# ZijiaLewisLu/CVPR2025-DeCafNet

Hardware: AMD Instinct MI355X
Metric: clips/sec (grounding fwd, T=16384 D=1024) (higher is better)
Workload: dtype f32; 1 GPU; BASELINE configs[2]: T=16384 D=1024 full multi-scale pyramid + sidekick top-k 30% + expert path, NQ=1 queries/video, 24 independent videos per step: 3 forwards in flight on 3 HIP streams x 8 videos per forward, one replica of this per GPU; T=16384, vid_len=16384, D=1024, E=256, TE=256, levels=8, win=9, heads=4, fusion_layers=2, sn=60, msf=True, norm=True, Lq=32, nq=1, max_batch=8, forwards_in_flight=3

## Files before the change

cvpr2025-decafnet_amd/_lib.py:

```python
import ctypes
import os

_HERE = os.path.dirname(os.path.abspath(__file__))
SO_PATH = os.environ.get('DCF_LIB_PATH') or os.path.join(_HERE, 'libdecafnet_hip.so')
_LIB = None

c_f32p = ctypes.c_void_p
c_u8p = ctypes.c_void_p
c_i32p = ctypes.c_void_p
c_i64p = ctypes.c_void_p
i32, i64, f32, f64 = ctypes.c_int32, ctypes.c_int64, ctypes.c_float, ctypes.c_double
vp = ctypes.c_void_p


class DcfConfig(ctypes.Structure):
    _fields_ = [(n, i32) for n in ('D', 'E', 'TE', 'vid_heads', 'fusion_heads', 'fusion_layers', 'n_embd_convs',
                                   'n_stem', 'n_levels', 'win', 'head_layers', 'sn')] + \
               [('sratio', f32)] + [(n, i32) for n in ('msf', 'norm', 'use_abs_pe', 'max_batch', 'gemm_mode', 'model_kind', 'second_fusion',
                                                      'text_in', 'text_layers', 'text_heads', 'text_abs_pe', 'text_bkgd',
                                                      'scat', 'sfonly', 'text_kind', 'xattn_affine', 'vid_stride', 'pool_only', 'attn_mode')]


SIGNATURES = {
    'dcf_last_error': (ctypes.c_char_p, []),
# ... 34 lines not shown
    'dcf_hybrid_phase2': (i32, [vp, c_f32p, c_u8p, i64, c_f32p, vp]),
    'dcf_hybrid_phase3': (i32, [vp, c_f32p, c_f32p, c_f32p, c_u8p, c_f32p, c_f32p, c_u8p, vp]),
    'dcf_debug_copy': (i32, [vp, i32, c_f32p, i64, vp]),
    'dcf_graph_active': (i32, [vp]),
    'dcf_debug_set_option': (i32, [ctypes.c_char_p, i32]),
    'dcf_calib_mfma_rate': (i32, [i32, i32, ctypes.POINTER(i32), ctypes.POINTER(f32)]),
    'dcf_model_set_graph_mode': (i32, [vp, i32]),
    'dcf_model_set_ln_carry': (i32, [vp, i32]),
    'dcf_profile_enable': (i32, [i32]),
    'dcf_profile_report': (i64, [ctypes.c_char_p, i64]),
    'dcf_collect_segments': (i32, [c_f32p, c_f32p, c_u8p, i32, i64, i32, f32, i32, f32, c_f32p, c_f32p, c_i32p, vp]),
    'dcf_collect_segments_ext': (i32, [c_f32p, c_f32p, c_u8p, c_f32p, i32, i64, i32, f32, i32, f32, c_f32p, c_f32p, c_i32p, vp]),
    'dcf_nms_1d': (i32, [c_f32p, c_f32p, c_i32p, i32, i32, i32, f32, c_i64p, c_i32p, vp]),
    'dcf_softnms_1d': (i32, [c_f32p, c_f32p, c_i32p, i32, i32, i32, f32, f32, f32, i32, i32, c_f32p, c_i64p, c_i32p, vp]),
    'dcf_segment_voting': (i32, [c_f32p, i32, c_i32p, i32, i32, c_f32p, c_f32p, c_i32p, i32, i32, f32, i32, c_f32p, vp]),
    'dcf_op_linear': (i32, [c_f32p, c_f32p, c_f32p, c_f32p, i32, i32, i32, i32, vp]),
    'dcf_op_linear_split': (i32, [c_f32p, c_f32p, c_f32p, c_f32p, i32, i32, i32, i32, i32, vp]),
    'dcf_op_linear_cm': (i32, [c_f32p, c_f32p, c_f32p, c_f32p, i32, i32, i32, vp]),
    'dcf_op_linear_ln': (i32, [c_f32p, c_f32p, c_f32p, c_f32p, c_f32p, c_f32p, c_f32p, i32, i32, i32, i32, i32, vp]),
    'dcf_op_linear_ln_carry': (i32, [c_f32p, c_f32p, c_f32p, c_f32p, c_f32p, c_f32p, c_f32p, c_f32p, c_f32p, c_f32p, i32, i32, i32, i32, i32, i32, vp]),
    'dcf_op_ffn': (i32, [c_f32p, c_f32p, c_f32p, c_f32p, c_f32p, c_f32p, c_f32p, c_f32p, c_u8p, c_f32p, c_f32p, i32, i32, i32, vp]),
    'dcf_op_linear_cm_split': (i32, [c_f32p, c_f32p, c_f32p, c_f32p, i32, i32, i32, i32, vp]),
    'dcf_op_head': (i32, [c_f32p, c_u8p, c_f32p, c_f32p, c_f32p, c_f32p, c_f32p, c_f32p, c_f32p, c_f32p, c_f32p, i32, i32, i32, i32, f32, i32, vp]),
    'dcf_op_conv3': (i32, [c_f32p, c_u8p, c_f32p, c_f32p, i32, i32, i32, i32, vp]),
    'dcf_op_conv3_split': (i32, [c_f32p, c_u8p, c_f32p, c_f32p, i32, i32, i32, i32, i32, vp]),
    'dcf_op_layernorm': (i32, [c_f32p, c_f32p, c_f32p, c_f32p, i32, i32, i32, vp]),
    'dcf_op_xattn': (i32, [c_f32p, c_f32p, c_f32p, c_u8p, c_f32p, i32, i32, i32, i32, i32, vp]),
    'dcf_op_local_attn': (i32, [c_f32p, c_f32p, c_f32p, c_u8p, c_f32p, i32, i32, i32, i32, i32, vp]),
    'dcf_op_sidekick': (i32, [c_f32p, c_f32p, c_f32p, i32, i32, i32, i32, vp]),
    'dcf_op_gate': (i32, [c_f32p, c_u8p, c_f32p, c_u8p, i32, i32, i32, f64, i32, vp]),
    'dcf_op_encoder': (i32, [vp, ctypes.c_char_p, c_f32p, c_u8p, i32, i32, i32, c_f32p, c_u8p, vp]),
    'dcf_op_enc_pre': (i32, [vp, ctypes.c_char_p, c_f32p, c_u8p, i32, i32, i32, c_f32p, c_f32p, c_f32p, c_f32p, vp]),
    'dcf_op_decoder': (i32, [vp, ctypes.c_char_p, c_f32p, c_u8p, i32, i32, ctypes.POINTER(vp), ctypes.POINTER(vp), ctypes.POINTER(i32), vp]),
    'dcf_op_tcn': (i32, [vp, ctypes.c_char_p, c_f32p, c_u8p, i32, i32, i32, i32, c_f32p, vp]),
}


def lib():
    global _LIB
    if _LIB is None:
        import torch
        if not os.path.exists(SO_PATH):
            raise RuntimeError(f'{SO_PATH} is missing: build it with __graft_entry__.build() '
                               f'(there is no CPU fallback for the grounding path)')
        h = ctypes.CDLL(SO_PATH, mode=ctypes.RTLD_GLOBAL)
        for name, (res, args) in SIGNATURES.items():
# ... 21 lines not shown
```

cvpr2025-decafnet_amd/csrc/engine.hip:

```cpp
#include <cstdarg>
#include <cstdio>
#include <cstdlib>
#include <algorithm>
#include <cstring>
#include <string>
#include <atomic>
#include <mutex>
#include <unordered_map>
#include <vector>

#include "../../include/decafnet_hip.h"
#include "attn.h"
#include "common.h"
#include "dec_chain.h"
#include "dropout.h"
#include "enc_chain.h"
#include "ffn_chain.h"
#include "gemm.h"
#include "head_chain.h"
#include "heads.h"
#include "postproc.h"
#include "rowops.h"
#include "score.h"

// ... 126 lines not shown
  const float *fc_wf, *fc_s, *fc_c;
  const unsigned short* qkv_chain[3];
  const float *qkv_s[3], *qkv_c[3];
  const unsigned short* wp_chain;
};
struct DecW {
  const float *ln_q_w, *ln_q_b, *ln_kv_w, *ln_kv_b, *dw, *qn_w, *qn_b;
  const float *wq, *bq, *wk, *bk, *wv, *bv, *wp, *bp;
  const float *wp_il, *bp_il;
  const float *ln_ffn_w, *ln_ffn_b, *fc_w, *fc_b, *pj_w, *pj_b, *ls_ffn;
  const float *fc_wf, *fc_s, *fc_c;
  const unsigned short *wq_chain, *wp_chain;
};
struct TextEncW {
  const float *ln_attn_w, *ln_attn_b, *wq, *bq, *wk, *bk, *wv, *bv, *wp, *bp, *ls_attn;
  const float *ln_ffn_w, *ln_ffn_b, *fc_w, *fc_b, *pj_w, *pj_b, *ls_ffn;
};
struct HeadW {
  std::vector<const float*> conv;
  std::vector<const float*> ln_w, ln_b;
  const float* out_w;
  const float* out_b;
  const unsigned short* chain[2] = {nullptr, nullptr};
};

static inline int vid_stride_of(const dcf_config& c) { return c.vid_stride > 1 ? c.vid_stride : 1; }

struct Plan {
  int T0 = 0, B = 0, L = 0;
  LevelTable lt{};
  LevelTable* d_lt = nullptr;
};

}

using namespace dcf;

namespace dcf { struct HybridState; }
using dcf::HybridState;

struct dcf_model {
  dcf_config cfg{};
  std::unordered_map<std::string, Bound> bound;
  std::vector<float*> owned;
  std::unordered_map<const float*, const unsigned short*> wsplit;
  std::unordered_map<const float*, int64_t> wsplit_ldw;
// ... 294 lines not shown
  for (int i = 0; i < layers; ++i) {
    const std::string s = std::to_string(i);
    GET(p + ".convs." + s + ".conv.weight", SH(C, C, 3), t);
    const float* pk;
    if (pack3(m, t, C, C, 3, 0, 2, 1, st, &pk)) return -1;
    SPLIT(pk, C, 3 * C);
    h.conv.push_back(pk);
    const float *lw, *lb;
    GET(p + ".norms." + s + ".weight", SH(C), lw); GET(p + ".norms." + s + ".bias", SH(C), lb);
    h.ln_w.push_back(lw); h.ln_b.push_back(lb);
  }
  GET(p + "." + out_name + ".conv.weight", SH(NO, C, 3), t);
  if (pack3(m, t, NO, C, 3, 0, 2, 1, st, &h.out_w)) return -1;
  GET(p + "." + out_name + ".conv.bias", SH(NO), h.out_b);
  h.chain[0] = h.chain[1] = nullptr;
  if (m->gemm_terms == GEMM_F16X3 && layers == 2 && head_chain_supports(C, NO)) {
    for (int i = 0; i < 2; ++i) {
      unsigned short* img = nullptr;
      DCF_HIP(hipMalloc(&img, head_chain_image_halfs(C) * sizeof(unsigned short)));
      m->owned.push_back(reinterpret_cast<float*>(img));
      if (launch_split_chain3(h.conv[i], img, C, st, nullptr)) return -1;
      h.chain[i] = img;
    }
  }
  return 0;
}

static inline bool vidmap_sfonly(const dcf_config& c) { return c.model_kind == 0 && c.msf && c.sfonly; }
static inline int vidmap_in_dim(const dcf_config& c) {
  return ((c.msf && !vidmap_sfonly(c)) ? 2 * c.D : c.D) + (c.scat ? 1 : 0);
}

static int finalize(dcf_model* m, hipStream_t st) {
  const dcf_config& c = m->cfg;
  const int E = c.E, D = c.D, TE = c.TE, L = c.n_levels;
  const bool sfonly = vidmap_sfonly(c);
  const int Din = vidmap_in_dim(c);
  for (float* p : m->owned) (void)hipFree(p);
  m->owned.clear();
  m->wsplit.clear();
  m->wsplit_ldw.clear();
  m->wsplit_terms.clear();
  if (init_gemm_mode(m, st)) return -1;
  m->dec.clear(); m->stem.clear(); m->branch.clear();
  m->embd_conv.clear(); m->embd_ln_w.clear(); m->embd_ln_b.clear();
  m->cls1 = HeadW(); m->cls2 = HeadW(); m->reg = HeadW();
// ... 403 lines not shown
  }
  GemmArgs gp = gemm(b.R[0], E, w.wp, w.bp, b.R[1], E, rows, E, E);
  gp.flags = G_RES | G_RES_MASK; gp.rowmask = mask_out; gp.ls = w.ls_attn;
  if (stride == 2) { gp.R = b.R[3]; gp.ldr = E; } else { gp.R = Xin; gp.ldr = ldx; }
  GemmArgs go = gemm(b.HID, 4 * E, w.pj_w, w.pj_b, Xout, ldo, rows, E, 4 * E);
  go.flags = G_RES | G_OUT_MASK; go.rowmask = mask_out; go.ls = w.ls_ffn; go.R = b.R[1]; go.ldr = E;
  if (can_fuse_ln(m, w.wp, rows, E, E, A_ROWS)) {
    gp.ln_w = w.ln_ffn_w; gp.ln_b = w.ln_ffn_b; gp.Y = b.R[2]; gp.ldy = E;
    TRY(run_gemm(m, &gp, 1, A_ROWS, st));
  } else if (can_carry_ln(m, w.wp, w.fc_wf, rows, E, E, E)) {
    gp.stats_out = b.stats; gp.stats_w = STATS_W;
    TRY(run_gemm(m, &gp, 1, A_ROWS, st));
    return run_ffn(m, b.R[1], w.fc_wf, w.fc_c, go, b.HID, rows, E, st, b.stats, w.fc_s);
  } else {
    TRY(run_gemm(m, &gp, 1, A_ROWS, st));
    LnArgs ln{}; ln.X = b.R[1]; ln.ldx = E; ln.Y = b.R[2]; ln.ldy = E; ln.w = w.ln_ffn_w; ln.b = w.ln_ffn_b; ln.rows = rows; ln.C = E;
    TRY(launch_ln(ln, st));
  }
  TRY(run_ffn(m, b.R[2], w.fc_w, w.fc_b, go, b.HID, rows, E, st));
  return 0;
}

static int head_chain_min_rows() {
  static const int v = getenv("DCF_HEAD_CHAIN_MIN_ROWS") ? atoi(getenv("DCF_HEAD_CHAIN_MIN_ROWS")) : 30000;
  return v;
}
static bool g_no_head_chain() {
  static const bool off = getenv("DCF_NO_HEAD_CHAIN") != nullptr;
  return off;
}
static bool can_chain_head(dcf_model* m, const HeadW& h, int rows, int Cin, int NO) {
  if (g_no_head_chain() || rows < head_chain_min_rows() || m->gemm_terms != GEMM_F16X3 || !h.chain[0] || !h.chain[1]) return false;
  if (h.conv.size() != 2 || !head_chain_supports(Cin, NO)) return false;
  for (int i = 0; i < 2; ++i)
    if (!m->wsplit.count(h.conv[i]) || m->wsplit_terms[h.conv[i]] != GEMM_F16X3) return false;
  return true;
}
static HeadChainArgs head_chain_args(dcf_model* m, const HeadW& h, Buffers& b, const Plan& pl, int NO, int mode, int query_major, float* out) {
  HeadChainArgs a{};
  a.X = b.F; a.ldx = m->cfg.E + TCN_HID; a.nbr = b.nbr_all; a.W1c = h.chain[0]; a.W2c = h.chain[1];
  a.ln1_w = h.ln_w[0]; a.ln1_b = h.ln_b[0]; a.ln2_w = h.ln_w[1]; a.ln2_b = h.ln_b[1];
  a.Wout = h.out_w; a.bout = h.out_b; a.lt = pl.d_lt; a.out = out; a.rows = pl.B * pl.lt.S; a.NO = NO; a.mode = mode;
  a.query_major = query_major; a.status = m->status;
  return a;
}
static int run_head_chain(dcf_model* m, const HeadChainArgs* a, int count, int Cin, hipStream_t st) {
  double flops = 0., bytes = 0.;
  for (int i = 0; i < count; ++i) {
    flops += 2.0 * a[i].rows * Cin * 3.0 * Cin * 2.0 + 2.0 * a[i].rows * 3.0 * Cin * a[i].NO;
    bytes += (double)a[i].rows * (Cin + a[i].NO) * 4.0;
  }
  ProfScope prof("gemm_f16x3<head_chain>", st, flops, bytes);
  return launch_head_chain(a, count, Cin, st);
}

static int run_head(dcf_model* m, const HeadW& h, Buffers& b, const Plan& pl, int Cin, int NO, int mode, int query_major,
                    float* out, hipStream_t st, int row0 = 0, int rows = -1) {
  if (row0 == 0 && rows < 0 && can_chain_head(m, h, pl.B * pl.lt.S, Cin, NO)) {
    const HeadChainArgs a = head_chain_args(m, h, b, pl, NO, mode, query_major, out);
    return run_head_chain(m, &a, 1, Cin, st);
  }
  const int rowsAll = rows >= 0 ? rows : pl.B * pl.lt.S;
  const int ldf = m->cfg.E + TCN_HID;
  const float* in = b.F + (int64_t)row0 * ldf;
  int64_t ldin = ldf;
// ... 1217 lines not shown
}

int dcf_hybrid_phase2(dcf_model* m, const float* featk_c, const uint8_t* maskk_c, int64_t off_k, float* refk_out, void* stream) {
  DCF_CHECK(m && featk_c && maskk_c && refk_out, "dcf_hybrid_phase2: null argument");
  DCF_CHECK(m->hyb && m->hyb->valid, "dcf_hybrid_phase2: no phase 1 on this model (or another forward ran since)");
  DCF_CHECK(off_k >= 0 && off_k + (m->hyb->Tn >> m->hyb->k) <= m->hyb->Tc, "dcf_hybrid_phase2: the narrow window must lie inside the coarse one");
  return dcf::hybrid_phase2(m, featk_c, maskk_c, (int)off_k, refk_out, (hipStream_t)stream);
}

int dcf_hybrid_phase3(dcf_model* m, const float* refk_c, float* logits_n, float* offsets_n, uint8_t* masks_n, float* logits_c,
                      float* offsets_c, uint8_t* masks_c, void* stream) {
  DCF_CHECK(m && refk_c && logits_n && offsets_n && masks_n, "dcf_hybrid_phase3: null argument");
  DCF_CHECK(m->hyb && m->hyb->valid, "dcf_hybrid_phase3: no phase 1 / 2 on this model (or another forward ran since)");
  DCF_CHECK(m->cfg.n_levels - m->hyb->k <= 1 || (logits_c && offsets_c && masks_c), "dcf_hybrid_phase3: null coarse outputs");
  const int rc = dcf::hybrid_phase3(m, refk_c, logits_n, offsets_n, masks_n, logits_c, offsets_c, masks_c, (hipStream_t)stream);
  m->hyb->valid = false;
  return rc;
}

int dcf_graph_active(const dcf_model* m) { return m ? m->last_launch : 0; }

int dcf_debug_set_option(const char* name, int32_t value) {
  DCF_CHECK(name && *name, "dcf_debug_set_option: empty name");
  static const char* known[] = {"dec_chain_min_rows", "enc_chain_min_rows", "enc_attn_min_rows", "fuse_scores", "tcn_frag", "gate_skip", "tcn_stack"};
  bool ok = false;
  for (const char* k : known) ok = ok || strcmp(k, name) == 0;
  DCF_CHECK(ok, "dcf_debug_set_option: unknown option '%s'", name);
  {
    std::lock_guard<std::mutex> lock(dcf::debug_options_mutex());
    if (value < 0) dcf::debug_options().erase(name);
    else dcf::debug_options()[name] = value;
  }
  dcf::g_option_epoch.fetch_add(1);
  return 0;
}

int dcf_model_set_graph_mode(dcf_model* m, int32_t mode) {
  DCF_CHECK(m && mode >= 0 && mode <= 2, "dcf_model_set_graph_mode: mode must be 0 (auto), 1 (always) or 2 (never)");
  if (mode != m->graph_mode) dcf::drop_graph(m);
  m->graph_mode = mode;
  return 0;
}

int dcf_debug_copy(dcf_model* m, int32_t what, float* dst, int64_t max_floats, void* stream) {
  DCF_CHECK(m && dst, "dcf_debug_copy: null argument");
  hipStream_t st = (hipStream_t)stream;
  const float* src = nullptr;
// ... 372 lines not shown
      dcf::GemmArgs g = dcf::gemm(in, C, wp[i], nullptr, bufs[i], C, rows, C, 3 * C);
      g.cin = C; g.nbr = nbr; g.Ws = img[i];
      rc = dcf::launch_gemm_split(&g, 1, dcf::A_ROWS_TAP3, nterms, st);
      if (rc == 0) {
        dcf::LnArgs ln{}; ln.X = bufs[i]; ln.ldx = C; ln.Y = bufs[i]; ln.ldy = C; ln.w = lw[i]; ln.b = lb[i]; ln.rows = rows; ln.C = C; ln.relu = 1;
        rc = dcf::launch_ln(ln, st);
      }
      in = bufs[i];
    }
    if (rc == 0) {
      dcf::ConvOutArgs co{};
      co.X = in; co.ldx = C; co.nbr = nbr; co.W = wo; co.bias = bout; co.lt = d_lt; co.out = out; co.rows = rows; co.C = C; co.NO = NO;
      co.row0 = 0; co.mode = mode; co.query_major = 0;
      rc = dcf::launch_conv_out(co, st);
    }
  }
  for (int i = 0; i < 2; ++i) { if (wp[i]) DCF_HIP(hipFreeAsync(wp[i], st)); if (img[i]) DCF_HIP(hipFreeAsync(img[i], st)); }
  if (ha) DCF_HIP(hipFreeAsync(ha, st));
  if (hb) DCF_HIP(hipFreeAsync(hb, st));
  DCF_HIP(hipFreeAsync(wo, st)); DCF_HIP(hipFreeAsync(nbr, st)); DCF_HIP(hipFreeAsync(d_lt, st));
  return rc;
}

int dcf_op_layernorm(const float* X, const float* w, const float* b, float* Y, int32_t rows, int32_t C, int32_t relu,
                     void* stream) {
  dcf::LnArgs a{};
  a.X = X; a.ldx = C; a.Y = Y; a.ldy = C; a.w = w; a.b = b; a.rows = rows; a.C = C; a.relu = relu;
  return dcf::launch_ln(a, (hipStream_t)stream);
}

int dcf_op_xattn(const float* Q, const float* K, const float* V, const uint8_t* kvmask, float* O, int32_t B, int32_t T,
                 int32_t Lk, int32_t C, int32_t heads, void* stream) {
  dcf::XAttnArgs a{Q, K, V, kvmask, O, B, T, Lk, C, heads};
  return dcf::launch_xattn(a, (hipStream_t)stream);
}

int dcf_op_local_attn(const float* Q, const float* K, const float* V, const uint8_t* mask, float* O, int32_t B, int32_t T,
                      int32_t C, int32_t heads, int32_t window, void* stream) {
  if (window == 0) {
    dcf::GlobalAttnArgs g{Q, K, V, mask, O, B, T, C, heads};
    return dcf::launch_global_attn(g, (hipStream_t)stream);
  }
  dcf::LocalAttnArgs a{Q, K, V, mask, O, B, T, C, heads, window};
  return dcf::launch_local_attn(a, (hipStream_t)stream);
}

// ... 150 lines not shown
```

cvpr2025-decafnet_amd/csrc/head_chain.h:

```cpp
#pragma once
#include <hip/hip_runtime.h>
#include <stdint.h>

#include "heads.h"

namespace dcf {

struct HeadChainArgs {
  const float* X;
  int64_t ldx;
  const uint8_t* nbr;
  const unsigned short* W1c;
  const unsigned short* W2c;
  const float* ln1_w; const float* ln1_b; const float* ln2_w; const float* ln2_b;
  const float* Wout;
  const float* bout;
  const LevelTable* lt;
  float* out;
  int rows, NO;
  int mode;
  int query_major;
  unsigned* status;
};

bool head_chain_supports(int C, int NO);
int launch_head_chain(const HeadChainArgs* a, int count, int C, hipStream_t stream);
size_t head_chain_image_halfs(int C);
int launch_split_chain3(const float* Wp, unsigned short* img, int C, hipStream_t stream, unsigned* overflow = nullptr);

}
```

cvpr2025-decafnet_amd/csrc/head_chain.hip:

```cpp
#include "head_chain.h"

#include <type_traits>

#include "common.h"

namespace dcf {

namespace {

typedef _Float16 f16x8 __attribute__((ext_vector_type(8)));
typedef _Float16 f16x2 __attribute__((ext_vector_type(2)));
typedef float f32x2 __attribute__((ext_vector_type(2)));
typedef unsigned u32x4 __attribute__((ext_vector_type(4)));

constexpr float SA = 16.f, SW = 256.f, UNSCALE = 1.f / 4096.f;
constexpr int HALO = 3, WGROWS = 128, VALID = WGROWS - 2 * HALO;

template <int C>
struct Geo {
  static constexpr int KS = C / 16;
  static constexpr int KH = KS / 2;
  static constexpr int NT = C / 32;
  static constexpr int PIECES = 3 * KH * 2;
  static constexpr int STAGE = PIECES * 1024;
  static constexpr int SPL = 2 * NT;
  static constexpr int NPW = (PIECES + 3) / 4;
  static_assert(C % 32 == 0 && KS % 2 == 0, "C must be a multiple of 32");
};

__device__ __forceinline__ void split2_f16(float x0, float x1, float s, unsigned& hi, unsigned& lo) {
  const f16x2 h = __builtin_convertvector(f32x2{x0 * s, x1 * s}, f16x2);
  hi = __builtin_bit_cast(unsigned, h);
  const float r0 = __builtin_fmaf(x0, s, -(float)h[0]), r1 = __builtin_fmaf(x1, s, -(float)h[1]);
  lo = __builtin_bit_cast(unsigned, __builtin_convertvector(f32x2{r0, r1}, f16x2));
}

__device__ __forceinline__ void glds16(const void* sbase, unsigned voff, unsigned lds_dst) {
#ifdef DCF_GLDS_KEEP_M0
  unsigned keep;
// ... 33 lines not shown

}

template <int C>
__global__ void k_split_chain3(const float* __restrict__ Wp, unsigned short* __restrict__ img, unsigned* __restrict__ overflow) {
  using G = Geo<C>;
  const int i = blockIdx.x * blockDim.x + threadIdx.x;
  if (i >= C * 3 * (C / 2)) return;
  const int n = i / (3 * (C / 2)), rem = i - n * (3 * (C / 2)), tap = rem / (C / 2), k = (rem - tap * (C / 2)) * 2;
  const float w0 = Wp[((size_t)n * 3 + tap) * C + k], w1 = Wp[((size_t)n * 3 + tap) * C + k + 1];
  unsigned hi, lo;
  split2_f16(w0, w1, SW, hi, lo);
  if (!(__builtin_fabsf(w0) * SW <= 65504.f) || !(__builtin_fabsf(w1) * SW <= 65504.f)) {
    if (overflow) atomicOr(overflow, 1u);
  }
  const int ot = n >> 5, rr = n & 31, kk = k >> 4, hf = kk / G::KH, kq = kk - hf * G::KH, kr = k & 15;
  const int a = kr >> 3, h = (kr >> 2) & 1, ii = kr & 3, j = 4 * a + ii;
  const size_t piece = (size_t)(ot * 2 + hf) * G::PIECES + (size_t)(tap * G::KH + kq) * 2;
  const size_t o = (piece * 64 + h * 32 + rr) * 8 + j;
  *reinterpret_cast<unsigned*>(img + o) = hi;
  *reinterpret_cast<unsigned*>(img + o + 64 * 8) = lo;
}

struct HeadChainBatch { HeadChainArgs a[2]; };
template <int C>
__global__ __launch_bounds__(256, 1) void k_head_chain(HeadChainBatch batch) {
  constexpr int NO = 2;
  const HeadChainArgs& p = batch.a[blockIdx.y];
  using G = Geo<C>;
  constexpr int KS = G::KS, KH = G::KH, NT = G::NT, STAGE = G::STAGE, PIECES = G::PIECES, NPW = G::NPW;
  extern __shared__ __attribute__((aligned(16))) unsigned char lds[];
  float* lds_ln = reinterpret_cast<float*>(lds + 2 * STAGE);
  float* lds_wo = lds_ln + 4 * C;
  float* lds_x = lds_wo + NO * 3 * C;
  const int tid = threadIdx.x, lane = tid & 63, r = lane & 31, h = lane >> 5;
  const int w = __builtin_amdgcn_readfirstlane(tid >> 6);
  const unsigned lane16 = (unsigned)lane * 16u;
  auto xch = [&](int par, int wave, int dir) __attribute__((always_inline)) -> float* { return lds_x + (((par * 4 + wave) * 2 + dir) * 2 + h) * 16; };
  const int wr = w * 32 + r;
  const int row = (int)blockIdx.x * VALID - HALO + wr;
  const bool inr = row >= 0 && row < p.rows;
  const int row_c = row < 0 ? 0 : (row < p.rows ? row : p.rows - 1);
  const unsigned fl = inr ? p.nbr[row_c] : 0u;
  const float sfl = (fl & 1u) ? UNSCALE : 0.f;
  const float lfl_in = ((fl & 2u) && r != 0) ? UNSCALE : 0.f, rfl_in = ((fl & 4u) && r != 31) ? UNSCALE : 0.f;
  const float lfl_x = ((fl & 2u) && r == 0 && w > 0) ? UNSCALE : 0.f, rfl_x = ((fl & 4u) && r == 31 && w < 3) ? UNSCALE : 0.f;
  const float lfl1 = (fl & 2u) ? 1.f : 0.f, rfl1 = (fl & 4u) ? 1.f : 0.f, sfl1 = (fl & 1u) ? 1.f : 0.f;

  auto issue_piece = [&](const unsigned short* img, int sl, int parity, int i) __attribute__((always_inline)) {
    int pc = w + 4 * i;
    pc = pc < PIECES ? pc : PIECES - 1;
#ifndef DCF_HC_NO_DMA
    glds16(img + ((size_t)sl * PIECES + pc) * 512, lane16, (unsigned)parity * STAGE + (unsigned)pc * 1024u);
#endif
  };
#ifdef DCF_HC_STAMP
  unsigned long long acc_[8] = {0, 0, 0, 0, 0, 0, 0, 0}, last_ = hc_stamp();
#endif
#pragma unroll
  for (int i = 0; i < NPW; ++i) issue_piece(p.W1c, 0, 0, i);

  for (int i = tid; i < C; i += 256) {
    lds_ln[i] = p.ln1_w[i]; lds_ln[C + i] = p.ln1_b[i]; lds_ln[2 * C + i] = p.ln2_w[i]; lds_ln[3 * C + i] = p.ln2_b[i];
  }
  for (int i = tid; i < NO * 3 * C; i += 256) lds_wo[i] = i < p.NO * 3 * C ? p.Wout[i] : 0.f;

  constexpr int XA = (256 - 16 * NT - 96) / 8 - 1 > 0 ? (256 - 16 * NT - 96) / 8 - 1 : 0;
  f16x8 xh[KS], xl[KS];
  {
    const float* px = p.X + (int64_t)row_c * p.ldx + 4 * h;
    const bool use = (fl & 1u) != 0;
#pragma unroll
    for (int kk = 0; kk < KS; ++kk) {
#ifndef DCF_HC_NO_X
      f32x4 v0 = *reinterpret_cast<const f32x4*>(px + 16 * kk), v1 = *reinterpret_cast<const f32x4*>(px + 16 * kk + 8);
#else
      f32x4 v0 = f32x4{0.1f, 0.2f, 0.3f, (float)lane}, v1 = f32x4{0.5f, (float)kk, 0.7f, 0.8f};
      (void)px;
#endif
      if (!use) { v0 = f32x4{0.f, 0.f, 0.f, 0.f}; v1 = v0; }
      unsigned hi[4], lo[4];
      split2_f16(v0.x, v0.y, SA, hi[0], lo[0]);
      split2_f16(v0.z, v0.w, SA, hi[1], lo[1]);
      split2_f16(v1.x, v1.y, SA, hi[2], lo[2]);
      split2_f16(v1.z, v1.w, SA, hi[3], lo[3]);
      xh[kk] = __builtin_bit_cast(f16x8, u32x4{hi[0], hi[1], hi[2], hi[3]});
      xl[kk] = __builtin_bit_cast(f16x8, u32x4{lo[0], lo[1], lo[2], lo[3]});
      if (kk < XA) { asm volatile("" : "+a"(xh[kk])); asm volatile("" : "+a"(xl[kk])); }
// ... 195 lines not shown
    }
  }

  STAMP(4);
  float pt[3][NO];
#pragma unroll
  for (int t = 0; t < 3; ++t)
#pragma unroll
    for (int o = 0; o < NO; ++o) pt[t][o] = 0.f;
#pragma unroll
  for (int ot = 0; ot < NT; ++ot)
#pragma unroll
    for (int g4 = 0; g4 < 4; ++g4)
#pragma unroll
      for (int o = 0; o < NO; ++o)
#pragma unroll
        for (int t = 0; t < 3; ++t) {
          const f32x4 wv = *reinterpret_cast<const f32x4*>(lds_wo + (o * 3 + t) * C + 32 * ot + 8 * g4 + 4 * h);
          pt[t][o] += (Y[ot][4 * g4] * wv.x + Y[ot][4 * g4 + 1] * wv.y) + (Y[ot][4 * g4 + 2] * wv.z + Y[ot][4 * g4 + 3] * wv.w);
        }
  float d0[NO], d1[NO], d2[NO];
#pragma unroll
  for (int o = 0; o < NO; ++o) { d0[o] = xor32_sum(pt[0][o]); d1[o] = xor32_sum(pt[1][o]); d2[o] = xor32_sum(pt[2][o]); }
  __syncthreads();
  if (h == 0) {
#pragma unroll
    for (int o = 0; o < NO; ++o) {
      if (r == 31) lds_x[(w * 2 + 0) * 2 + o] = d0[o];
      if (r == 0) lds_x[(w * 2 + 1) * 2 + o] = d2[o];
    }
  }
  __syncthreads();
  float yo[NO];
#pragma unroll
  for (int o = 0; o < NO; ++o) {
    const float xl_ = lds_x[((w > 0 ? w - 1 : 0) * 2 + 0) * 2 + o], xr_ = lds_x[((w < 3 ? w + 1 : 3) * 2 + 1) * 2 + o];
    const float sp = from_prev(d0[o]), sn = from_next(d2[o]);
    const float pv = r == 0 ? (w > 0 ? xl_ : 0.f) : sp;
    const float nx = r == 31 ? (w < 3 ? xr_ : 0.f) : sn;
    yo[o] = __builtin_fmaf(pv, lfl1, __builtin_fmaf(nx, rfl1, d1[o] * sfl1)) + (o < p.NO ? p.bout[o] : 0.f);
  }
  if (h == 0 && wr >= HALO && wr < HALO + VALID && inr) {
    const LevelTable* lt = p.lt;
    const int l = find_level_hc(lt, row);
    int64_t dst = row;
    if (p.query_major) {
      const int rel = row - lt->start[l];
      const int b = rel / lt->T[l], t = rel - b * lt->T[l];
      dst = (int64_t)b * lt->S + lt->off[l] + t;
    }
#pragma unroll
    for (int o = 0; o < NO; ++o) {
      float y = yo[o];
      if (p.mode == 1) y = fmaxf(y * lt->scale[l], 0.f);
      if (o < p.NO) p.out[dst * p.NO + o] = y;
    }
  }
  if (bad && p.status) atomicOr(p.status, 1u);
#ifdef DCF_HC_STAMP
  STAMP(6);
#ifndef DCF_HC_STAMP_WG
#define DCF_HC_STAMP_WG 1
#endif
  if (blockIdx.x == DCF_HC_STAMP_WG && blockIdx.y == 0 && tid == 0)
    for (int i = 0; i < 8; ++i) dcf_hc_stamps[i] = acc_[i];
#endif
}

#ifdef DCF_HC_STAMP
}
extern "C" int dcf_debug_hc_stamps(unsigned long long* out) {
  return hipMemcpyFromSymbol(out, HIP_SYMBOL(dcf::dcf_hc_stamps), 8 * sizeof(unsigned long long)) == hipSuccess ? 0 : -1;
}
namespace dcf {
#endif

bool head_chain_supports(int C, int NO) { return (C == 256 || C == 288) && (NO == 1 || NO == 2); }

size_t head_chain_image_halfs(int C) { return (size_t)(C / 32) * 2 * (3 * (C / 32) * 2) * 512; }

int launch_split_chain3(const float* Wp, unsigned short* img, int C, hipStream_t stream, unsigned* overflow) {
  DCF_CHECK(C == 256 || C == 288, "launch_split_chain3: C = %d (256 or 288)", C);
  const int n = C * 3 * (C / 2);
  if (C == 256) hipLaunchKernelGGL(k_split_chain3<256>, dim3((n + 255) / 256), dim3(256), 0, stream, Wp, img, overflow);
  else hipLaunchKernelGGL(k_split_chain3<288>, dim3((n + 255) / 256), dim3(256), 0, stream, Wp, img, overflow);
  DCF_HIP(hipGetLastError());
  return 0;
}

template <int C>
static int launch_hc(const HeadChainArgs* a, int count, hipStream_t stream) {
  constexpr int bytes = 2 * Geo<C>::STAGE + (4 * C + 2 * 3 * C + 2 * 4 * 2 * 2 * 16) * (int)sizeof(float);
  static bool attr_set[64] = {};
  int dev = 0;
  DCF_HIP(hipGetDevice(&dev));
  if (dev >= 0 && dev < 64 && !attr_set[dev]) {
    DCF_HIP(hipFuncSetAttribute(reinterpret_cast<const void*>(&k_head_chain<C>), hipFuncAttributeMaxDynamicSharedMemorySize, bytes));
    attr_set[dev] = true;
  }
  HeadChainBatch b{};
  for (int i = 0; i < count; ++i) b.a[i] = a[i];
  const unsigned grid = (unsigned)((a[0].rows + VALID - 1) / VALID);
  hipLaunchKernelGGL((k_head_chain<C>), dim3(grid, (unsigned)count), dim3(256), bytes, stream, b);
  DCF_HIP(hipGetLastError());
  return 0;
}

int launch_head_chain(const HeadChainArgs* a, int count, int C, hipStream_t stream) {
  DCF_CHECK(count == 1 || count == 2, "launch_head_chain: one or two heads per launch");
  for (int i = 0; i < count; ++i) {
    DCF_CHECK(head_chain_supports(C, a[i].NO), "launch_head_chain: C = %d, NO = %d (C 256 / 288, NO 1 / 2)", C, a[i].NO);
    DCF_CHECK(a[i].rows > 0 && a[i].rows == a[0].rows && a[i].X && a[i].nbr && a[i].W1c && a[i].W2c && a[i].ln1_w && a[i].ln1_b && a[i].ln2_w &&
                  a[i].ln2_b && a[i].Wout && a[i].bout && a[i].lt && a[i].out, "launch_head_chain: null argument or unequal row counts");
    DCF_CHECK((reinterpret_cast<uintptr_t>(a[i].X) & 15) == 0 && a[i].ldx % 4 == 0 && (reinterpret_cast<uintptr_t>(a[i].W1c) & 15) == 0 &&
                  (reinterpret_cast<uintptr_t>(a[i].W2c) & 15) == 0, "launch_head_chain: X / weight images must be 16-byte aligned");
  }
  return C == 256 ? launch_hc<256>(a, count, stream) : launch_hc<288>(a, count, stream);
}

}
```

include/decafnet_hip.h:

```cpp
#ifndef DECAFNET_HIP_H
#define DECAFNET_HIP_H

#include <stdint.h>

#ifdef __cplusplus
extern "C" {
#endif

const char* dcf_last_error(void);
int dcf_abi_version(void);

typedef struct dcf_model dcf_model;

typedef struct dcf_config {
  int32_t D;
  int32_t E;
  int32_t TE;
  int32_t vid_heads;
  int32_t fusion_heads;
  int32_t fusion_layers;
  int32_t n_embd_convs;
  int32_t n_stem;
  int32_t n_levels;
  int32_t win;
// ... 126 lines not shown

int dcf_op_linear(const float* A, const float* W, const float* bias, float* C, int32_t M, int32_t N, int32_t K,
                  int32_t act, void* stream);
int dcf_op_linear_split(const float* A, const float* W, const float* bias, float* C, int32_t M, int32_t N, int32_t K,
                        int32_t act, int32_t nterms, void* stream);
int dcf_op_linear_cm(const float* A_cm, const float* W, const float* bias, float* C, int32_t M, int32_t N, int32_t K,
                     void* stream);
int dcf_op_linear_ln(const float* A, const float* W, const float* bias, const float* ln_w, const float* ln_b, float* C, float* Y,
                     int32_t M, int32_t N, int32_t K, int32_t relu, int32_t nterms, void* stream);

int dcf_op_linear_ln_carry(const float* A, const float* W1, const float* b1, const float* R, const float* ln_w, const float* ln_b,
                           const float* W2, const float* b2, float* X, float* Y, int32_t M, int32_t N1, int32_t K1, int32_t N2,
                           int32_t gelu, int32_t nterms, void* stream);

int dcf_op_ffn(const float* X, const float* ln_w, const float* ln_b, const float* W1, const float* b1, const float* W2, const float* b2,
               const float* ls, const uint8_t* mask, float* C, float* stats_out, int32_t M, int32_t E, int32_t chain, void* stream);

int dcf_op_linear_cm_split(const float* A_cm, const float* W, const float* bias, float* C, int32_t M, int32_t N, int32_t K,
                           int32_t nterms, void* stream);
int dcf_op_head(const float* X, const uint8_t* mask, const float* W1, const float* ln1_w, const float* ln1_b, const float* W2,
                const float* ln2_w, const float* ln2_b, const float* Wout, const float* bout, float* out, int32_t B, int32_t T,
                int32_t C, int32_t NO, float scale, int32_t chain, void* stream);

int dcf_op_conv3(const float* X, const uint8_t* mask, const float* W_ock, float* Y, int32_t B, int32_t T, int32_t Cin,
                 int32_t N, void* stream);
int dcf_op_conv3_split(const float* X, const uint8_t* mask, const float* W_ock, float* Y, int32_t B, int32_t T, int32_t Cin,
                       int32_t N, int32_t nterms, void* stream);
int dcf_op_layernorm(const float* X, const float* w, const float* b, float* Y, int32_t rows, int32_t C, int32_t relu,
                     void* stream);
int dcf_op_xattn(const float* Q, const float* K, const float* V, const uint8_t* kvmask, float* O, int32_t B, int32_t T,
                 int32_t Lk, int32_t C, int32_t heads, void* stream);
int dcf_op_local_attn(const float* Q, const float* K, const float* V, const uint8_t* mask, float* O, int32_t B, int32_t T,
                      int32_t C, int32_t heads, int32_t window, void* stream);
int dcf_op_sidekick(const float* shallow, const float* text_cls, float* correl, int32_t D, int32_t T, int32_t nq,
                    int32_t norm, void* stream);
int dcf_op_gate(const float* correl, const uint8_t* vid_mask, float* gate, uint8_t* mask_out, int32_t T, int32_t nq,
                int32_t sn, double sratio, int32_t msf, void* stream);

int dcf_op_encoder(dcf_model* m, const char* prefix, const float* X, const uint8_t* mask, int32_t B, int32_t T, int32_t stride,
                   float* Y, uint8_t* mask_out, void* stream);
int dcf_op_enc_pre(dcf_model* m, const char* prefix, const float* X, const uint8_t* mask, int32_t B, int32_t T, int32_t stride,
                   float* Qc, float* Kc, float* Vc, float* Skip, void* stream);
int dcf_op_decoder(dcf_model* m, const char* prefix, float* X, const uint8_t* mask, int32_t B, int32_t T,
                   const float* const* text, const uint8_t* const* text_mask, const int32_t* text_len, void* stream);
int dcf_op_tcn(dcf_model* m, const char* prefix, const float* x, const uint8_t* mask, int32_t B, int32_t T, int32_t n_in,
               int32_t n_layers, float* Y, void* stream);
// ... 6 lines not shown
```

Measured before the change: 21.52 million clips/s.

## Template head chain on output count and pre-pack head parameters into one image

The fused head-chain kernel is templated on the number of outputs, so the classification and regression heads get separate specialised bodies instead of both padding to two outputs. LayerNorm weights, the output conv and its bias are packed once at finalize into a contiguous image that is streamed into LDS with async global-to-LDS loads instead of scalar copies. Each row's output index and level scale are worked out before the main loop and kept in LDS, which removes the level search from the epilogue. The halo exchange now uses a double buffer, dropping one barrier, and a standalone pyramid-head entry point is added for testing.

New measurement: 21.68 million clips/s, median of 6. Within noise of the previous version (+0.7%).

```diff
diff --git a/cvpr2025-decafnet_amd/_lib.py b/cvpr2025-decafnet_amd/_lib.py
--- a/cvpr2025-decafnet_amd/_lib.py
+++ b/cvpr2025-decafnet_amd/_lib.py
@@ -80,6 +80,8 @@
     'dcf_op_ffn': (i32, [c_f32p, c_f32p, c_f32p, c_f32p, c_f32p, c_f32p, c_f32p, c_f32p, c_u8p, c_f32p, c_f32p, i32, i32, i32, vp]),
     'dcf_op_linear_cm_split': (i32, [c_f32p, c_f32p, c_f32p, c_f32p, i32, i32, i32, i32, vp]),
     'dcf_op_head': (i32, [c_f32p, c_u8p, c_f32p, c_f32p, c_f32p, c_f32p, c_f32p, c_f32p, c_f32p, c_f32p, c_f32p, i32, i32, i32, i32, f32, i32, vp]),
+    'dcf_op_head_pyramid': (i32, [c_f32p, c_u8p, c_f32p, c_f32p, c_f32p, c_f32p, c_f32p, c_f32p, c_f32p, c_f32p, c_f32p, c_f32p, i32, i32,
+                                  ctypes.POINTER(i32), ctypes.POINTER(f32), i32, i32, i32, i32, vp]),
     'dcf_op_conv3': (i32, [c_f32p, c_u8p, c_f32p, c_f32p, i32, i32, i32, i32, vp]),
     'dcf_op_conv3_split': (i32, [c_f32p, c_u8p, c_f32p, c_f32p, i32, i32, i32, i32, i32, vp]),
     'dcf_op_layernorm': (i32, [c_f32p, c_f32p, c_f32p, c_f32p, i32, i32, i32, vp]),
diff --git a/cvpr2025-decafnet_amd/csrc/engine.hip b/cvpr2025-decafnet_amd/csrc/engine.hip
--- a/cvpr2025-decafnet_amd/csrc/engine.hip
+++ b/cvpr2025-decafnet_amd/csrc/engine.hip
@@ -172,6 +172,7 @@
   const float* out_w;
   const float* out_b;
   const unsigned short* chain[2] = {nullptr, nullptr};
+  const float* params = nullptr;
 };
 
 static inline int vid_stride_of(const dcf_config& c) { return c.vid_stride > 1 ? c.vid_stride : 1; }
@@ -512,6 +513,11 @@
       if (launch_split_chain3(h.conv[i], img, C, st, nullptr)) return -1;
       h.chain[i] = img;
     }
+    float* pimg = nullptr;
+    DCF_HIP(hipMalloc(&pimg, head_chain_param_floats(C, NO) * sizeof(float)));
+    m->owned.push_back(pimg);
+    if (launch_head_params(h.ln_w[0], h.ln_b[0], h.ln_w[1], h.ln_b[1], h.out_w, h.out_b, pimg, C, NO, st)) return -1;
+    h.params = pimg;
   }
   return 0;
 }
@@ -961,6 +967,8 @@
 }
 
 static int head_chain_min_rows() {
+  const int o = debug_option("head_chain_min_rows", -1);
+  if (o >= 0) return o;
   static const int v = getenv("DCF_HEAD_CHAIN_MIN_ROWS") ? atoi(getenv("DCF_HEAD_CHAIN_MIN_ROWS")) : 30000;
   return v;
 }
@@ -979,7 +987,7 @@
   HeadChainArgs a{};
   a.X = b.F; a.ldx = m->cfg.E + TCN_HID; a.nbr = b.nbr_all; a.W1c = h.chain[0]; a.W2c = h.chain[1];
   a.ln1_w = h.ln_w[0]; a.ln1_b = h.ln_b[0]; a.ln2_w = h.ln_w[1]; a.ln2_b = h.ln_b[1];
-  a.Wout = h.out_w; a.bout = h.out_b; a.lt = pl.d_lt; a.out = out; a.rows = pl.B * pl.lt.S; a.NO = NO; a.mode = mode;
+  a.Wout = h.out_w; a.bout = h.out_b; a.params = h.params; a.lt = pl.d_lt; a.out = out; a.rows = pl.B * pl.lt.S; a.NO = NO; a.mode = mode;
   a.query_major = query_major; a.status = m->status;
   return a;
 }
@@ -2243,7 +2251,7 @@
 
 int dcf_debug_set_option(const char* name, int32_t value) {
   DCF_CHECK(name && *name, "dcf_debug_set_option: empty name");
-  static const char* known[] = {"dec_chain_min_rows", "enc_chain_min_rows", "enc_attn_min_rows", "fuse_scores", "tcn_frag", "gate_skip", "tcn_stack"};
+  static const char* known[] = {"head_chain_min_rows", "dec_chain_min_rows", "enc_chain_min_rows", "enc_attn_min_rows", "fuse_scores", "tcn_frag", "gate_skip", "tcn_stack"};
   bool ok = false;
   for (const char* k : known) ok = ok || strcmp(k, name) == 0;
   DCF_CHECK(ok, "dcf_debug_set_option: unknown option '%s'", name);
@@ -2662,6 +2670,59 @@
   return rc;
 }
 
+int dcf_op_head_pyramid(const float* X, const uint8_t* mask, const float* W1, const float* ln1_w, const float* ln1_b, const float* W2,
+                        const float* ln2_w, const float* ln2_b, const float* Wout, const float* bout, const float* params, float* out,
+                        int32_t B, int32_t n_levels, const int32_t* T, const float* scales, int32_t C, int32_t NO, int32_t mode,
+                        int32_t query_major, void* stream) {
+  hipStream_t st = (hipStream_t)stream;
+  DCF_CHECK(X && mask && W1 && W2 && out && T && scales && B > 0 && n_levels >= 1 && n_levels <= dcf::DCF_MAX_LEVELS, "dcf_op_head_pyramid: null argument or level count");
+  DCF_CHECK(params || (ln1_w && ln1_b && ln2_w && ln2_b && Wout && bout), "dcf_op_head_pyramid: neither a parameter image nor the six parameter arrays");
+  DCF_CHECK(dcf::head_chain_supports(C, NO) && (mode == 0 || mode == 1), "dcf_op_head_pyramid: C = %d (256 / 288), NO = %d (1 / 2), mode = %d (0 / 1)", C, NO, mode);
+  dcf::LevelTable lt{}, *d_lt = nullptr;
+  lt.n_levels = n_levels; lt.B = B;
+  int S = 0;
+  for (int l = 0; l < n_levels; ++l) {
+    DCF_CHECK(T[l] > 0, "dcf_op_head_pyramid: T[%d] = %d", l, T[l]);
+    lt.T[l] = T[l]; lt.start[l] = B * S; lt.off[l] = S; lt.scale[l] = scales[l];
+    S += T[l];
+  }
+  lt.S = S; lt.start[n_levels] = B * S;
+  const int rows = B * S;
+  float *wp[2] = {nullptr, nullptr}, *wo = nullptr;
+  unsigned short* img[2] = {nullptr, nullptr};
+  uint8_t* nbr = nullptr;
+  DCF_HIP(hipMallocAsync((void**)&d_lt, sizeof(lt), st));
+  DCF_HIP(hipMemcpyAsync(d_lt, &lt, sizeof(lt), hipMemcpyHostToDevice, st));
+  DCF_HIP(hipStreamSynchronize(st));
+  DCF_HIP(hipMallocAsync((void**)&nbr, (size_t)rows, st));
+  int rc = 0;
+  for (int l = 0; l < n_levels && rc == 0; ++l) rc = dcf::launch_rowflags(mask + lt.start[l], nbr + lt.start[l], T[l], B * T[l], st);
+  const float* Ws[2] = {W1, W2};
+  for (int i = 0; i < 2 && rc == 0; ++i) {
+    DCF_HIP(hipMallocAsync((void**)&wp[i], (size_t)C * C * 3 * sizeof(float), st));
+    DCF_HIP(hipMallocAsync((void**)&img[i], dcf::head_chain_image_halfs(C) * sizeof(unsigned short), st));
+    const int n = C * C * 3;
+    hipLaunchKernelGGL(dcf::k_permute3, dim3((n + 255) / 256), dim3(256), 0, st, Ws[i], wp[i], C, C, 3, 0, 2, 1);
+    rc = dcf::launch_split_chain3(wp[i], img[i], C, st);
+  }
+  if (rc == 0 && !params) {
+    const int n = NO * C * 3;
+    DCF_HIP(hipMallocAsync((void**)&wo, (size_t)n * sizeof(float), st));
+    hipLaunchKernelGGL(dcf::k_permute3, dim3((n + 255) / 256), dim3(256), 0, st, Wout, wo, NO, C, 3, 0, 2, 1);
+  }
+  if (rc == 0) {
+    dcf::HeadChainArgs a{};
+    a.X = X; a.ldx = C; a.nbr = nbr; a.W1c = img[0]; a.W2c = img[1]; a.params = params;
+    if (!params) { a.ln1_w = ln1_w; a.ln1_b = ln1_b; a.ln2_w = ln2_w; a.ln2_b = ln2_b; a.Wout = wo; a.bout = bout; }
+    a.lt = d_lt; a.out = out; a.rows = rows; a.NO = NO; a.mode = mode; a.query_major = query_major;
+    rc = dcf::launch_head_chain(&a, 1, C, st);
+  }
+  for (int i = 0; i < 2; ++i) { if (wp[i]) DCF_HIP(hipFreeAsync(wp[i], st)); if (img[i]) DCF_HIP(hipFreeAsync(img[i], st)); }
+  if (wo) DCF_HIP(hipFreeAsync(wo, st));
+  DCF_HIP(hipFreeAsync(nbr, st)); DCF_HIP(hipFreeAsync(d_lt, st));
+  return rc;
+}
+
 int dcf_op_layernorm(const float* X, const float* w, const float* b, float* Y, int32_t rows, int32_t C, int32_t relu,
                      void* stream) {
   dcf::LnArgs a{};
diff --git a/cvpr2025-decafnet_amd/csrc/head_chain.h b/cvpr2025-decafnet_amd/csrc/head_chain.h
--- a/cvpr2025-decafnet_amd/csrc/head_chain.h
+++ b/cvpr2025-decafnet_amd/csrc/head_chain.h
@@ -15,6 +15,7 @@
   const float* ln1_w; const float* ln1_b; const float* ln2_w; const float* ln2_b;
   const float* Wout;
   const float* bout;
+  const float* params;
   const LevelTable* lt;
   float* out;
   int rows, NO;
@@ -25,6 +26,9 @@
 
 bool head_chain_supports(int C, int NO);
 int launch_head_chain(const HeadChainArgs* a, int count, int C, hipStream_t stream);
+size_t head_chain_param_floats(int C, int NO);
+int launch_head_params(const float* ln1_w, const float* ln1_b, const float* ln2_w, const float* ln2_b, const float* Wout, const float* bout,
+                       float* img, int C, int NO, hipStream_t stream);
 size_t head_chain_image_halfs(int C);
 int launch_split_chain3(const float* Wp, unsigned short* img, int C, hipStream_t stream, unsigned* overflow = nullptr);
 
diff --git a/cvpr2025-decafnet_amd/csrc/head_chain.hip b/cvpr2025-decafnet_amd/csrc/head_chain.hip
--- a/cvpr2025-decafnet_amd/csrc/head_chain.hip
+++ b/cvpr2025-decafnet_amd/csrc/head_chain.hip
@@ -1,5 +1,6 @@
 #include "head_chain.h"
 
+#include <cstdlib>
 #include <type_traits>
 
 #include "common.h"
@@ -15,6 +16,9 @@
 
 constexpr float SA = 16.f, SW = 256.f, UNSCALE = 1.f / 4096.f;
 constexpr int HALO = 3, WGROWS = 128, VALID = WGROWS - 2 * HALO;
+
+constexpr int XCH_FLOATS = 2 * 4 * 2 * 2 * 16;
+constexpr int param_floats(int C, int NO) { return (4 * C + NO * 3 * C + NO + 255) / 256 * 256; }
 
 template <int C>
 struct Geo {
@@ -94,17 +98,18 @@
   *reinterpret_cast<unsigned*>(img + o + 64 * 8) = lo;
 }
 
-struct HeadChainBatch { HeadChainArgs a[2]; };
-template <int C>
-__global__ __launch_bounds__(256, 1) void k_head_chain(HeadChainBatch batch) {
-  constexpr int NO = 2;
-  const HeadChainArgs& p = batch.a[blockIdx.y];
+template <int C, int NO>
+__device__ __forceinline__ void head_chain_body(const HeadChainArgs& p) {
   using G = Geo<C>;
   constexpr int KS = G::KS, KH = G::KH, NT = G::NT, STAGE = G::STAGE, PIECES = G::PIECES, NPW = G::NPW;
+  constexpr int PF = param_floats(C, NO), NPP = PF / 256;
   extern __shared__ __attribute__((aligned(16))) unsigned char lds[];
   float* lds_ln = reinterpret_cast<float*>(lds + 2 * STAGE);
   float* lds_wo = lds_ln + 4 * C;
-  float* lds_x = lds_wo + NO * 3 * C;
+  const float* lds_bo = lds_wo + NO * 3 * C;
+  float* lds_x = lds_ln + PF;
+  int* lds_dst = reinterpret_cast<int*>(lds_x + XCH_FLOATS);
+  float* lds_sc = reinterpret_cast<float*>(lds_dst + WGROWS);
   const int tid = threadIdx.x, lane = tid & 63, r = lane & 31, h = lane >> 5;
   const int w = __builtin_amdgcn_readfirstlane(tid >> 6);
   const unsigned lane16 = (unsigned)lane * 16u;
@@ -129,13 +134,34 @@
 #ifdef DCF_HC_STAMP
   unsigned long long acc_[8] = {0, 0, 0, 0, 0, 0, 0, 0}, last_ = hc_stamp();
 #endif
+  {
+    const LevelTable* lt = p.lt;
+    const int nl = lt->n_levels;
+    int st_ = lt->start[0], T_ = lt->T[0], off_ = lt->off[0];
+    float sc_ = lt->scale[0];
+#pragma unroll 1
+    for (int l = 1; l < nl; ++l) {
+      const int s_l = lt->start[l], t_l = lt->T[l], o_l = lt->off[l];
+      const float c_l = lt->scale[l];
+      const bool in = row >= s_l;
+      st_ = in ? s_l : st_; T_ = in ? t_l : T_; off_ = in ? o_l : off_; sc_ = in ? c_l : sc_;
+    }
+    int dst = row;
+    if (p.query_major) {
+      const int rel = row - st_, td = T_ > 0 ? T_ : 1;
+      const int b = rel / td, t = rel - b * td;
+      dst = b * lt->S + off_ + t;
+    }
+    if (h == 0) { lds_dst[wr] = dst; lds_sc[wr] = sc_; }
+  }
 #pragma unroll
   for (int i = 0; i < NPW; ++i) issue_piece(p.W1c, 0, 0, i);
 
-  for (int i = tid; i < C; i += 256) {
-    lds_ln[i] = p.ln1_w[i]; lds_ln[C + i] = p.ln1_b[i]; lds_ln[2 * C + i] = p.ln2_w[i]; lds_ln[3 * C + i] = p.ln2_b[i];
-  }
-  for (int i = tid; i < NO * 3 * C; i += 256) lds_wo[i] = i < p.NO * 3 * C ? p.Wout[i] : 0.f;
+#pragma unroll
+  for (int i = 0; i < (NPP + 3) / 4; ++i) {
+    const int pc = w + 4 * i;
+    if (pc < NPP) glds16(p.params + pc * 256, lane16, 2u * STAGE + (unsigned)pc * 1024u);
+  }
 
   constexpr int XA = (256 - 16 * NT - 96) / 8 - 1 > 0 ? (256 - 16 * NT - 96) / 8 - 1 : 0;
   f16x8 xh[KS], xl[KS];
@@ -377,38 +403,32 @@
   float d0[NO], d1[NO], d2[NO];
 #pragma unroll
   for (int o = 0; o < NO; ++o) { d0[o] = xor32_sum(pt[0][o]); d1[o] = xor32_sum(pt[1][o]); d2[o] = xor32_sum(pt[2][o]); }
-  __syncthreads();
+  float* ox = lds_x + (NT & 1) * (XCH_FLOATS / 2);
   if (h == 0) {
 #pragma unroll
     for (int o = 0; o < NO; ++o) {
-      if (r == 31) lds_x[(w * 2 + 0) * 2 + o] = d0[o];
-      if (r == 0) lds_x[(w * 2 + 1) * 2 + o] = d2[o];
+      if (r == 31) ox[(w * 2 + 0) * NO + o] = d0[o];
+      if (r == 0) ox[(w * 2 + 1) * NO + o] = d2[o];
     }
   }
   __syncthreads();
   float yo[NO];
 #pragma unroll
   for (int o = 0; o < NO; ++o) {
-    const float xl_ = lds_x[((w > 0 ? w - 1 : 0) * 2 + 0) * 2 + o], xr_ = lds_x[((w < 3 ? w + 1 : 3) * 2 + 1) * 2 + o];
+    const float xl_ = ox[((w > 0 ? w - 1 : 0) * 2 + 0) * NO + o], xr_ = ox[((w < 3 ? w + 1 : 3) * 2 + 1) * NO + o];
     const float sp = from_prev(d0[o]), sn = from_next(d2[o]);
     const float pv = r == 0 ? (w > 0 ? xl_ : 0.f) : sp;
     const float nx = r == 31 ? (w < 3 ? xr_ : 0.f) : sn;
-    yo[o] = __builtin_fmaf(pv, lfl1, __builtin_fmaf(nx, rfl1, d1[o] * sfl1)) + (o < p.NO ? p.bout[o] : 0.f);
+    yo[o] = __builtin_fmaf(pv, lfl1, __builtin_fmaf(nx, rfl1, d1[o] * sfl1)) + lds_bo[o];
   }
   if (h == 0 && wr >= HALO && wr < HALO + VALID && inr) {
-    const LevelTable* lt = p.lt;
-    const int l = find_level_hc(lt, row);
-    int64_t dst = row;
-    if (p.query_major) {
-      const int rel = row - lt->start[l];
-      const int b = rel / lt->T[l], t = rel - b * lt->T[l];
-      dst = (int64_t)b * lt->S + lt->off[l] + t;
-    }
+    const int64_t dst = lds_dst[wr];
+    const float sc = lds_sc[wr];
 #pragma unroll
     for (int o = 0; o < NO; ++o) {
       float y = yo[o];
-      if (p.mode == 1) y = fmaxf(y * lt->scale[l], 0.f);
-      if (o < p.NO) p.out[dst * p.NO + o] = y;
+      if (p.mode == 1) y = fmaxf(y * sc, 0.f);
+      p.out[dst * NO + o] = y;
     }
   }
   if (bad && p.status) atomicOr(p.status, 1u);
@@ -420,6 +440,33 @@
   if (blockIdx.x == DCF_HC_STAMP_WG && blockIdx.y == 0 && tid == 0)
     for (int i = 0; i < 8; ++i) dcf_hc_stamps[i] = acc_[i];
 #endif
+}
+
+struct HeadChainBatch { HeadChainArgs a[2]; };
+template <int C, int NO>
+__global__ __launch_bounds__(256, 1) void k_head_chain(HeadChainBatch batch) {
+  head_chain_body<C, NO>(batch.a[blockIdx.y]);
+}
+template <int C, int NO0, int NO1>
+__global__ __launch_bounds__(256, 1) void k_head_chain2(HeadChainBatch batch) {
+  if (blockIdx.y == 0) head_chain_body<C, NO0>(batch.a[0]);
+  else head_chain_body<C, NO1>(batch.a[1]);
+}
+
+__global__ void k_pack_head_params(const float* __restrict__ ln1_w, const float* __restrict__ ln1_b, const float* __restrict__ ln2_w,
+                                   const float* __restrict__ ln2_b, const float* __restrict__ Wout, const float* __restrict__ bout,
+                                   float* __restrict__ img, int C, int NO, int total) {
+  const int i = blockIdx.x * blockDim.x + threadIdx.x;
+  if (i >= total) return;
+  const int nw = NO * 3 * C;
+  float v = 0.f;
+  if (i < C) v = ln1_w[i];
+  else if (i < 2 * C) v = ln1_b[i - C];
+  else if (i < 3 * C) v = ln2_w[i - 2 * C];
+  else if (i < 4 * C) v = ln2_b[i - 3 * C];
+  else if (i < 4 * C + nw) v = Wout[i - 4 * C];
+  else if (i < 4 * C + nw + NO) v = bout[i - 4 * C - nw];
+  img[i] = v;
 }
 
 #ifdef DCF_HC_STAMP
@@ -443,34 +490,84 @@
   return 0;
 }
 
-template <int C>
-static int launch_hc(const HeadChainArgs* a, int count, hipStream_t stream) {
-  constexpr int bytes = 2 * Geo<C>::STAGE + (4 * C + 2 * 3 * C + 2 * 4 * 2 * 2 * 16) * (int)sizeof(float);
+size_t head_chain_param_floats(int C, int NO) { return (size_t)param_floats(C, NO); }
+
+int launch_head_params(const float* ln1_w, const float* ln1_b, const float* ln2_w, const float* ln2_b, const float* Wout, const float* bout,
+                       float* img, int C, int NO, hipStream_t stream) {
+  DCF_CHECK(head_chain_supports(C, NO) && ln1_w && ln1_b && ln2_w && ln2_b && Wout && bout && img, "launch_head_params: C = %d, NO = %d or a null argument", C, NO);
+  const int n = param_floats(C, NO);
+  hipLaunchKernelGGL(k_pack_head_params, dim3((n + 255) / 256), dim3(256), 0, stream, ln1_w, ln1_b, ln2_w, ln2_b, Wout, bout, img, C, NO, n);
+  DCF_HIP(hipGetLastError());
+  return 0;
+}
+
+template <int C, int NO>
+constexpr int hc_lds_bytes() { return 2 * Geo<C>::STAGE + (param_floats(C, NO) + XCH_FLOATS + 2 * WGROWS) * (int)sizeof(float); }
+
+template <auto kernel>
+static int launch_hc(int bytes, const HeadChainArgs* a, int count, hipStream_t stream) {
   static bool attr_set[64] = {};
   int dev = 0;
   DCF_HIP(hipGetDevice(&dev));
   if (dev >= 0 && dev < 64 && !attr_set[dev]) {
-    DCF_HIP(hipFuncSetAttribute(reinterpret_cast<const void*>(&k_head_chain<C>), hipFuncAttributeMaxDynamicSharedMemorySize, bytes));
+    DCF_HIP(hipFuncSetAttribute(reinterpret_cast<const void*>(kernel), hipFuncAttributeMaxDynamicSharedMemorySize, bytes));
     attr_set[dev] = true;
   }
   HeadChainBatch b{};
   for (int i = 0; i < count; ++i) b.a[i] = a[i];
   const unsigned grid = (unsigned)((a[0].rows + VALID - 1) / VALID);
-  hipLaunchKernelGGL((k_head_chain<C>), dim3(grid, (unsigned)count), dim3(256), bytes, stream, b);
+  hipLaunchKernelGGL(kernel, dim3(grid, (unsigned)count), dim3(256), bytes, stream, b);
   DCF_HIP(hipGetLastError());
   return 0;
 }
 
-int launch_head_chain(const HeadChainArgs* a, int count, int C, hipStream_t stream) {
+template <int C, int NO>
+static int launch_hc_same(const HeadChainArgs* a, int count, hipStream_t stream) {
+  return launch_hc<&k_head_chain<C, NO>>(hc_lds_bytes<C, NO>(), a, count, stream);
+}
+
+static bool pair_split() {
+  static const bool v = getenv("DCF_HEAD_PAIR_SPLIT") != nullptr;
+  return v;
+}
+
+int launch_head_chain(const HeadChainArgs* a_in, int count, int C, hipStream_t stream) {
   DCF_CHECK(count == 1 || count == 2, "launch_head_chain: one or two heads per launch");
+  HeadChainArgs a[2];
+  float* built[2] = {nullptr, nullptr};
   for (int i = 0; i < count; ++i) {
+    a[i] = a_in[i];
     DCF_CHECK(head_chain_supports(C, a[i].NO), "launch_head_chain: C = %d, NO = %d (C 256 / 288, NO 1 / 2)", C, a[i].NO);
-    DCF_CHECK(a[i].rows > 0 && a[i].rows == a[0].rows && a[i].X && a[i].nbr && a[i].W1c && a[i].W2c && a[i].ln1_w && a[i].ln1_b && a[i].ln2_w &&
-                  a[i].ln2_b && a[i].Wout && a[i].bout && a[i].lt && a[i].out, "launch_head_chain: null argument or unequal row counts");
+    DCF_CHECK(a[i].rows > 0 && a[i].rows == a[0].rows && a[i].X && a[i].nbr && a[i].W1c && a[i].W2c && a[i].lt && a[i].out &&
+                  (a[i].params || (a[i].ln1_w && a[i].ln1_b && a[i].ln2_w && a[i].ln2_b && a[i].Wout && a[i].bout)),
+              "launch_head_chain: null argument or unequal row counts");
     DCF_CHECK((reinterpret_cast<uintptr_t>(a[i].X) & 15) == 0 && a[i].ldx % 4 == 0 && (reinterpret_cast<uintptr_t>(a[i].W1c) & 15) == 0 &&
-                  (reinterpret_cast<uintptr_t>(a[i].W2c) & 15) == 0, "launch_head_chain: X / weight images must be 16-byte aligned");
-  }
-  return C == 256 ? launch_hc<256>(a, count, stream) : launch_hc<288>(a, count, stream);
-}
-
-}
+                  (reinterpret_cast<uintptr_t>(a[i].W2c) & 15) == 0 && (reinterpret_cast<uintptr_t>(a[i].params) & 15) == 0,
+              "launch_head_chain: X / weight / parameter images must be 16-byte aligned");
+  }
+  int rc = 0;
+  for (int i = 0; i < count && rc == 0; ++i) {
+    if (a[i].params) continue;
+    DCF_HIP(hipMallocAsync((void**)&built[i], head_chain_param_floats(C, a[i].NO) * sizeof(float), stream));
+    rc = launch_head_params(a[i].ln1_w, a[i].ln1_b, a[i].ln2_w, a[i].ln2_b, a[i].Wout, a[i].bout, built[i], C, a[i].NO, stream);
+    a[i].params = built[i];
+  }
+  auto one = [&](const HeadChainArgs* q, int n) {
+    if (C == 256) return q[0].NO == 1 ? launch_hc_same<256, 1>(q, n, stream) : launch_hc_same<256, 2>(q, n, stream);
+    return q[0].NO == 1 ? launch_hc_same<288, 1>(q, n, stream) : launch_hc_same<288, 2>(q, n, stream);
+  };
+  if (rc == 0) {
+    if (count == 1 || a[0].NO == a[1].NO) rc = one(a, count);
+    else if (C == 288 && a[0].NO == 1 && a[1].NO == 2 && !pair_split())
+      rc = launch_hc<&k_head_chain2<288, 1, 2>>(hc_lds_bytes<288, 2>(), a, 2, stream);
+    else {
+      rc = one(a, 1);
+      if (rc == 0) rc = one(a + 1, 1);
+    }
+  }
+  for (int i = 0; i < 2; ++i)
+    if (built[i]) DCF_HIP(hipFreeAsync(built[i], stream));
+  return rc;
+}
+
+}
diff --git a/include/decafnet_hip.h b/include/decafnet_hip.h
--- a/include/decafnet_hip.h
+++ b/include/decafnet_hip.h
@@ -172,6 +172,11 @@
                 const float* ln2_w, const float* ln2_b, const float* Wout, const float* bout, float* out, int32_t B, int32_t T,
                 int32_t C, int32_t NO, float scale, int32_t chain, void* stream);
 
+int dcf_op_head_pyramid(const float* X, const uint8_t* mask, const float* W1, const float* ln1_w, const float* ln1_b, const float* W2,
+                        const float* ln2_w, const float* ln2_b, const float* Wout, const float* bout, const float* params, float* out,
+                        int32_t B, int32_t n_levels, const int32_t* T, const float* scales, int32_t C, int32_t NO, int32_t mode,
+                        int32_t query_major, void* stream);
+
 int dcf_op_conv3(const float* X, const uint8_t* mask, const float* W_ock, float* Y, int32_t B, int32_t T, int32_t Cin,
                  int32_t N, void* stream);
 int dcf_op_conv3_split(const float* X, const uint8_t* mask, const float* W_ock, float* Y, int32_t B, int32_t T, int32_t Cin,
```
